# bqqbarbhg/rtk

Hardware: AMD Instinct MI355X
Metric: Mrays/sec (primary, closest-hit) on 1M-tri scene (higher is better)
Workload: dtype f32; 1 GPU; config2: 1M-tri soup (seed 1, spread 0.02), 4096x4096 coherent pinhole primary rays; bvh=gpu-lbvh, bvh_nodes=462584, launch=persistent, ray_order=as given, parallelism=ray-batch shards x1, BVH replicated

## Files before the change

include/rtk_amd.h:

```cpp
#ifndef RTK_AMD_H
#define RTK_AMD_H

#include "rtk.h"

#ifdef __cplusplus
extern "C" {
#endif

enum {
	RTK_AMD_OK = 0,
	RTK_AMD_ERR_NO_DEVICE = -1,
	RTK_AMD_ERR_BAD_ARG = -2,
	RTK_AMD_ERR_OOM = -3,
	RTK_AMD_ERR_HIP = -4,
	RTK_AMD_ERR_BAD_SCENE = -5,
	RTK_AMD_ERR_UNSUPPORTED = -6,
};

const char *rtk_amd_last_error(void);
int rtk_amd_device_count(void);
int rtk_amd_set_device(int device);

typedef struct rtk_dev_scene rtk_dev_scene;

// ... 137 lines not shown
typedef struct rtk_dev_filter {
	uint32_t struct_size;
	uint32_t mesh_mask_bits;
	const uint32_t *d_mesh_mask;
	const uint32_t *d_ignore_prim;
	const rtk_hit_record *d_after;
} rtk_dev_filter;
int rtk_dev_trace_rays_filtered(const rtk_dev_scene *ds, const rtk_ray *d_rays, size_t n,
	rtk_hit_record *d_hits, const rtk_dev_filter *filter, const rtk_trace_opts *opts, void *stream);
int rtk_dev_trace_rays_any_filtered(const rtk_dev_scene *ds, const rtk_ray *d_rays, size_t n,
	uint8_t *d_occluded, const rtk_dev_filter *filter, const rtk_trace_opts *opts, void *stream);
int rtk_dev_trace_status(const rtk_dev_scene *ds, void *stream);

int rtk_dev_detect_image(const rtk_dev_scene *ds, const rtk_ray *d_rays, size_t n, uint32_t *width, uint32_t *height, void *stream);

int rtk_dev_trace_rays_counted(const rtk_dev_scene *ds, const rtk_ray *d_rays, size_t n,
	rtk_hit_record *d_hits, const rtk_trace_opts *opts, rtk_trace_counters *out);

int rtk_dev_trace_rays_any_counted(const rtk_dev_scene *ds, const rtk_ray *d_rays, size_t n,
	uint8_t *d_occluded, const rtk_trace_opts *opts, rtk_trace_counters *out);

typedef struct rtk_packet_counters {
	uint64_t tiles;
	uint64_t pairs;
	uint64_t node_steps;
	uint64_t triangles_fetched;
	uint64_t triangle_group_tests;
	uint64_t tiles_handed_back;
	uint64_t handed_back_node_steps;
	uint64_t handed_back_triangle_steps;
} rtk_packet_counters;
int rtk_dev_trace_rays_packet_counted(const rtk_dev_scene *ds, const rtk_ray *d_rays, size_t n,
	rtk_hit_record *d_hits, const rtk_trace_opts *opts, rtk_packet_counters *out);

typedef struct rtk_mgpu rtk_mgpu;
void rtk_amd_shard_range(size_t n, int rank, int num_shards, size_t *first, size_t *count);
rtk_mgpu *rtk_mgpu_create(const int *devices, int num_devices);
void rtk_mgpu_destroy(rtk_mgpu *m);
int rtk_mgpu_num_devices(const rtk_mgpu *m);
const rtk_dev_scene *rtk_mgpu_scene(const rtk_mgpu *m, int index);
int rtk_mgpu_build(rtk_mgpu *m, const rtk_scene_desc *desc);
int rtk_mgpu_upload(rtk_mgpu *m, const rtk_scene *scene);
int rtk_mgpu_refit(rtk_mgpu *m, const rtk_scene_desc *desc);
int rtk_mgpu_refit_meshes(rtk_mgpu *m, const rtk_scene_desc *desc, const uint32_t *mesh_ids, size_t num_ids);
int rtk_mgpu_build_placed(rtk_mgpu *m, const rtk_scene_desc *desc, const rtk_placement *placements);
int rtk_mgpu_refit_placed(rtk_mgpu *m, const rtk_scene_desc *desc, const rtk_placement *placements);
int rtk_mgpu_refit_meshes_placed(rtk_mgpu *m, const rtk_scene_desc *desc, const rtk_placement *placements,
                                 const uint32_t *mesh_ids, size_t num_ids);
int rtk_mgpu_split_leaves(rtk_mgpu *m, uint32_t max_leaf);
int rtk_mgpu_rebuild(rtk_mgpu *m);
int rtk_mgpu_trace_rays(rtk_mgpu *m, const rtk_ray *rays, size_t n, rtk_hit_record *records, const rtk_trace_opts *opts);
int rtk_mgpu_trace_rays_device(rtk_mgpu *m, const rtk_ray *const *d_rays, const size_t *counts, rtk_hit_record *const *d_records,
	rtk_hit_record *d_gathered, int root_index, const rtk_trace_opts *opts);
int rtk_mgpu_trace_rays_device_striped(rtk_mgpu *m, const rtk_ray *const *d_rays, const size_t *counts, rtk_hit_record *const *d_records,
	rtk_hit_record *const *d_striped, const rtk_trace_opts *opts);
void rtk_mgpu_striped_segment(const size_t *counts, int num_shards, int shard, int stripe, size_t *first, size_t *count);

size_t rtk_trace_rays(const rtk_scene *scene, const rtk_ray *rays, size_t n, rtk_hit *hits, uint8_t *hit_mask);
size_t rtk_trace_rays_filter(const rtk_scene *scene, const rtk_ray *rays, size_t n, rtk_hit *hits, uint8_t *hit_mask,
	rtk_filter_fn *filter, void *filter_user);
void rtk_amd_forget_scene(const rtk_scene *scene);

#ifdef __cplusplus
}
#endif
#endif
// ... 1 lines not shown
```

rtk_amd/api.py:

```python
import ctypes as C
import os

import numpy as np

from .types import (HIT_DTYPE, HIT_RECORD_DTYPE, RAY_DTYPE, MeshSet, Placement, SceneDesc, SceneHeader, placement_array)

HERE = os.path.dirname(os.path.abspath(__file__))
LIB_PATH = os.environ.get("RTK_AMD_LIB") or os.path.join(HERE, "librtk_amd.so")

RTK_TRACE_STATIC = 1
RTK_TRACE_NO_PACKET = 2
RTK_TRACE_SORT_RAYS = 4
RTK_TRACE_EXACT_NODES = 8
RTK_TRACE_NO_ASM = 16


class RtkError(RuntimeError):
    pass


class SceneInfo(C.Structure):
    _fields_ = [("num_triangles", C.c_uint64), ("num_meshes", C.c_uint64), ("num_nodes", C.c_uint64),
                ("node_bytes", C.c_uint64), ("triangle_bytes", C.c_uint64), ("total_device_bytes", C.c_uint64),
                ("max_depth", C.c_uint32), ("stack_entries", C.c_uint32), ("build_ms", C.c_double)]
# ... 40 lines not shown


class TraceOpts(C.Structure):
    _fields_ = [("struct_size", C.c_uint32), ("flags", C.c_uint32), ("image_width", C.c_uint32),
                ("image_height", C.c_uint32), ("refill_min", C.c_uint32), ("blocks_per_cu", C.c_uint32),
                ("node_exit", C.c_uint32)]


class DevFilter(C.Structure):
    _fields_ = [("struct_size", C.c_uint32), ("mesh_mask_bits", C.c_uint32), ("d_mesh_mask", C.c_void_p),
                ("d_ignore_prim", C.c_void_p), ("d_after", C.c_void_p)]


FILTER_FN = C.CFUNCTYPE(C.c_bool, C.c_void_p, C.c_void_p, C.c_void_p)


class TraceCounters(C.Structure):
    _fields_ = [("rays", C.c_uint64), ("nodes", C.c_uint64), ("leaves", C.c_uint64),
                ("triangles", C.c_uint64), ("hits", C.c_uint64), ("stack_spills", C.c_uint64),
                ("wave_node_steps", C.c_uint64), ("wave_triangle_steps", C.c_uint64), ("wave_rays", C.c_uint64)]

    def as_dict(self):
        return {k: int(getattr(self, k)) for k, _ in self._fields_}


class PacketCounters(C.Structure):
    _fields_ = [("tiles", C.c_uint64), ("pairs", C.c_uint64), ("node_steps", C.c_uint64), ("triangles_fetched", C.c_uint64),
                ("triangle_group_tests", C.c_uint64), ("tiles_handed_back", C.c_uint64),
                ("handed_back_node_steps", C.c_uint64), ("handed_back_triangle_steps", C.c_uint64)]

    def as_dict(self):
        return {k: int(getattr(self, k)) for k, _ in self._fields_}


RTK_H_SYMBOLS = ["rtk_start_build", "rtk_run_task", "rtk_get_build_size", "rtk_finish_build_to",
                 "rtk_finish_build", "rtk_build_scene", "rtk_free_scene", "rtk_trace_ray", "rtk_trace_ray_filter"]
RTK_AMD_H_SYMBOLS = ["rtk_amd_last_error", "rtk_amd_device_count", "rtk_amd_set_device",
                     "rtk_dev_scene_upload", "rtk_dev_scene_build", "rtk_dev_scene_free", "rtk_dev_scene_get_info",
                     "rtk_dev_scene_mesh_base", "rtk_dev_scene_primitive_order", "rtk_dev_scene_export_size", "rtk_dev_scene_export",
                     "rtk_dev_trace_rays", "rtk_dev_trace_rays_any", "rtk_dev_expand_hits",
                     "rtk_dev_trace_rays_counted", "rtk_dev_trace_rays_any_counted", "rtk_dev_trace_rays_packet_counted", "rtk_dev_detect_image", "rtk_trace_rays", "rtk_amd_forget_scene",
                     "rtk_dev_scene_validate", "rtk_amd_release_workspace", "rtk_dev_scene_upload_buffer",
                     "rtk_dev_trace_rays_filtered", "rtk_dev_trace_rays_any_filtered", "rtk_dev_trace_status",
                     "rtk_trace_rays_filter", "rtk_amd_shard_range", "rtk_mgpu_create", "rtk_mgpu_destroy", "rtk_mgpu_num_devices",
                     "rtk_mgpu_scene", "rtk_mgpu_build", "rtk_mgpu_upload", "rtk_mgpu_trace_rays", "rtk_mgpu_trace_rays_device",
                     "rtk_amd_set_builder", "rtk_amd_get_builder", "rtk_amd_set_per_ray",
                     "rtk_mgpu_trace_rays_device_striped", "rtk_mgpu_striped_segment",
                     "rtk_dev_scene_refit", "rtk_dev_scene_last_refit_ms", "rtk_mgpu_refit",
                     "rtk_dev_scene_refit_meshes", "rtk_dev_scene_last_refit_nodes", "rtk_mgpu_refit_meshes",
                     "rtk_dev_scene_quality", "rtk_dev_scene_split_leaves", "rtk_mgpu_split_leaves",
                     "rtk_dev_scene_rebuild", "rtk_mgpu_rebuild",
                     "rtk_dev_scene_build_placed", "rtk_dev_scene_refit_placed", "rtk_dev_scene_refit_meshes_placed",
                     "rtk_mgpu_build_placed", "rtk_mgpu_refit_placed", "rtk_mgpu_refit_meshes_placed"]

_lib = None


def lib():
    global _lib
    if _lib is not None:
        return _lib
    if not os.path.exists(LIB_PATH):
        raise RtkError("%s not found: build it with `make -C rtk_amd/csrc` (or __graft_entry__.build()); "
                       "there is no CPU fallback" % LIB_PATH)
    import torch
    L = C.CDLL(LIB_PATH)
    L.rtk_amd_last_error.restype = C.c_char_p
    L.rtk_amd_device_count.restype = C.c_int
    L.rtk_amd_set_device.argtypes = [C.c_int]
    L.rtk_dev_scene_upload.restype = C.c_void_p
    L.rtk_dev_scene_upload.argtypes = [C.c_void_p]
    L.rtk_dev_scene_build.restype = C.c_void_p
    L.rtk_dev_scene_build.argtypes = [C.POINTER(SceneDesc)]
    L.rtk_dev_scene_free.argtypes = [C.c_void_p]
    L.rtk_dev_scene_get_info.argtypes = [C.c_void_p, C.POINTER(SceneInfo)]
    L.rtk_dev_scene_mesh_base.argtypes = [C.c_void_p, C.c_void_p, C.c_size_t]
    L.rtk_dev_scene_primitive_order.restype = C.c_longlong
    L.rtk_dev_scene_primitive_order.argtypes = [C.c_void_p, C.c_void_p, C.c_size_t]
    L.rtk_dev_scene_export_size.restype = C.c_size_t
    L.rtk_dev_scene_export_size.argtypes = [C.c_void_p]
    L.rtk_dev_scene_export.restype = C.c_void_p
    L.rtk_dev_scene_export.argtypes = [C.c_void_p, C.c_void_p, C.c_size_t]
    L.rtk_dev_trace_rays.argtypes = [C.c_void_p, C.c_void_p, C.c_size_t, C.c_void_p, C.POINTER(TraceOpts), C.c_void_p]
    L.rtk_dev_trace_rays_any.argtypes = [C.c_void_p, C.c_void_p, C.c_size_t, C.c_void_p, C.POINTER(TraceOpts), C.c_void_p]
    L.rtk_dev_expand_hits.argtypes = [C.c_void_p, C.c_void_p, C.c_size_t, C.c_void_p, C.c_void_p, C.c_void_p]
    L.rtk_dev_trace_rays_packet_counted.argtypes = [C.c_void_p, C.c_void_p, C.c_size_t, C.c_void_p, C.POINTER(TraceOpts), C.POINTER(PacketCounters)]
    L.rtk_dev_trace_rays_counted.argtypes = [C.c_void_p, C.c_void_p, C.c_size_t, C.c_void_p, C.POINTER(TraceOpts),
                                             C.POINTER(TraceCounters)]
    L.rtk_dev_trace_rays_any_counted.argtypes = [C.c_void_p, C.c_void_p, C.c_size_t, C.c_void_p, C.POINTER(TraceOpts),
                                                 C.POINTER(TraceCounters)]
    L.rtk_trace_rays.restype = C.c_size_t
    L.rtk_trace_rays.argtypes = [C.c_void_p, C.c_void_p, C.c_size_t, C.c_void_p, C.c_void_p]
    L.rtk_amd_forget_scene.argtypes = [C.c_void_p]
    L.rtk_dev_scene_validate.argtypes = [C.c_void_p, C.POINTER(SceneCheck)]
    L.rtk_dev_scene_upload_buffer.restype = C.c_void_p
    L.rtk_dev_scene_upload_buffer.argtypes = [C.c_void_p, C.c_size_t]
    L.rtk_dev_trace_rays_filtered.argtypes = [C.c_void_p, C.c_void_p, C.c_size_t, C.c_void_p, C.POINTER(DevFilter),
                                              C.POINTER(TraceOpts), C.c_void_p]
    L.rtk_dev_trace_rays_any_filtered.argtypes = [C.c_void_p, C.c_void_p, C.c_size_t, C.c_void_p, C.POINTER(DevFilter),
                                                  C.POINTER(TraceOpts), C.c_void_p]
    L.rtk_dev_trace_status.argtypes = [C.c_void_p, C.c_void_p]
    L.rtk_trace_rays_filter.restype = C.c_size_t
    L.rtk_trace_rays_filter.argtypes = [C.c_void_p, C.c_void_p, C.c_size_t, C.c_void_p, C.c_void_p, C.c_void_p, C.c_void_p]
    L.rtk_amd_shard_range.restype = None
    L.rtk_amd_shard_range.argtypes = [C.c_size_t, C.c_int, C.c_int, C.POINTER(C.c_size_t), C.POINTER(C.c_size_t)]
    L.rtk_mgpu_create.restype = C.c_void_p
    L.rtk_mgpu_create.argtypes = [C.POINTER(C.c_int), C.c_int]
    L.rtk_mgpu_destroy.restype = None
    L.rtk_mgpu_destroy.argtypes = [C.c_void_p]
    L.rtk_mgpu_num_devices.argtypes = [C.c_void_p]
    L.rtk_mgpu_scene.restype = C.c_void_p
    L.rtk_mgpu_scene.argtypes = [C.c_void_p, C.c_int]
    L.rtk_mgpu_build.argtypes = [C.c_void_p, C.POINTER(SceneDesc)]
    L.rtk_mgpu_upload.argtypes = [C.c_void_p, C.c_void_p]
    L.rtk_mgpu_refit.restype = C.c_int
    L.rtk_mgpu_refit.argtypes = [C.c_void_p, C.POINTER(SceneDesc)]
    L.rtk_dev_scene_refit.restype = C.c_int
    L.rtk_dev_scene_refit.argtypes = [C.c_void_p, C.POINTER(SceneDesc), C.c_void_p]
    L.rtk_dev_scene_last_refit_ms.restype = C.c_double
# ... 342 lines not shown
            d_rays = to_device(rays)
        d_occ = torch.empty(n, dtype=torch.uint8, device="cuda")
        ctr = TraceCounters()
        torch.cuda.synchronize()
        _check(lib().rtk_dev_trace_rays_any_counted(self.handle, C.c_void_p(d_rays.data_ptr()), n, C.c_void_p(d_occ.data_ptr()),
                                                    C.byref(opts) if opts is not None else None, C.byref(ctr)),
               "rtk_dev_trace_rays_any_counted")
        return d_occ.cpu().numpy().astype(bool), ctr.as_dict()

    def trace_counted(self, rays, opts=None):
        torch = _torch()
        if hasattr(rays, "data_ptr"):
            d_rays, n = rays, rays.numel() * rays.element_size() // 32
        else:
            rays = np.ascontiguousarray(rays)
            n = rays.shape[0]
            d_rays = to_device(rays)
        d_rec = torch.empty(n * 16, dtype=torch.uint8, device="cuda")
        ctr = TraceCounters()
        torch.cuda.synchronize()
        _check(lib().rtk_dev_trace_rays_counted(self.handle, C.c_void_p(d_rays.data_ptr()), n, C.c_void_p(d_rec.data_ptr()),
                                                C.byref(opts) if opts is not None else None, C.byref(ctr)),
               "rtk_dev_trace_rays_counted")
        return d_rec.cpu().numpy().view(HIT_RECORD_DTYPE), ctr.as_dict()


    def detect_image(self, rays):
        rays = np.ascontiguousarray(rays)
        d_rays = to_device(rays)
        w, h = C.c_uint32(0), C.c_uint32(0)
        _check(lib().rtk_dev_detect_image(self.handle, C.c_void_p(d_rays.data_ptr()), C.c_size_t(rays.shape[0]), C.byref(w), C.byref(h), _stream_ptr()), "rtk_dev_detect_image")
        return int(w.value), int(h.value)

    def trace_packet_counted(self, rays, opts):
        torch = _torch()
        if hasattr(rays, "data_ptr"):
            d_rays, n = rays, rays.numel() * rays.element_size() // 32
        else:
            rays = np.ascontiguousarray(rays)
            n = rays.shape[0]
            d_rays = to_device(rays)
        d_rec = torch.empty(n * 16, dtype=torch.uint8, device="cuda")
        ctr = PacketCounters()
        torch.cuda.synchronize()
        _check(lib().rtk_dev_trace_rays_packet_counted(self.handle, C.c_void_p(d_rays.data_ptr()), n, C.c_void_p(d_rec.data_ptr()),
                                                       C.byref(opts) if opts is not None else None, C.byref(ctr)),
               "rtk_dev_trace_rays_packet_counted")
        return d_rec.cpu().numpy().view(HIT_RECORD_DTYPE), ctr.as_dict()



def build_scene(meshes):
    _torch()
    ms = meshes if isinstance(meshes, MeshSet) else MeshSet(meshes)
    p = lib().rtk_build_scene(C.byref(ms.desc))
    if not p:
        raise RtkError("rtk_build_scene failed: " + last_error())
    return p, ms


def free_scene(scene_ptr):
    lib().rtk_free_scene(C.c_void_p(scene_ptr))


def scene_bytes(scene_ptr):
    hdr = SceneHeader.from_address(scene_ptr)
# ... 41 lines not shown
```

rtk_amd/csrc/rtk_capi.hip:

```cpp
#include "rtk_dev.h"
#include "rtk_trace_plan.h"

#include <algorithm>
#include "rtk_layout_check.h"

#include <stdarg.h>
#include <stdio.h>
#include <stdlib.h>
#include <string.h>

#include <chrono>
#include <atomic>
#include <mutex>
#include <unordered_map>


static thread_local char g_error[512] = "";

void rtk_set_error(const char *fmt, ...)
{
	va_list ap;
	va_start(ap, fmt);
	vsnprintf(g_error, sizeof(g_error), fmt, ap);
	va_end(ap);
// ... 107 lines not shown
}

extern "C" int rtk_dev_trace_rays_filtered(const rtk_dev_scene *ds, const rtk_ray *d_rays, size_t n,
	rtk_hit_record *d_hits, const rtk_dev_filter *filter, const rtk_trace_opts *opts, void *stream)
{
	return rtk_launch_trace(ds, d_rays, n, d_hits, nullptr, opts, (hipStream_t)stream, false, nullptr, filter);
}

extern "C" int rtk_dev_trace_rays_any_filtered(const rtk_dev_scene *ds, const rtk_ray *d_rays, size_t n,
	uint8_t *d_occluded, const rtk_dev_filter *filter, const rtk_trace_opts *opts, void *stream)
{
	return rtk_launch_trace(ds, d_rays, n, nullptr, d_occluded, opts, (hipStream_t)stream, true, nullptr, filter);
}

extern "C" int rtk_dev_trace_rays_counted(const rtk_dev_scene *ds, const rtk_ray *d_rays, size_t n,
	rtk_hit_record *d_hits, const rtk_trace_opts *opts, rtk_trace_counters *out)
{
	if (!out) { rtk_set_error("rtk_dev_trace_rays_counted: NULL counters"); return RTK_AMD_ERR_BAD_ARG; }
	return rtk_launch_trace(ds, d_rays, n, d_hits, nullptr, opts, nullptr, false, out);
}

extern "C" int rtk_dev_trace_rays_any_counted(const rtk_dev_scene *ds, const rtk_ray *d_rays, size_t n,
	uint8_t *d_occluded, const rtk_trace_opts *opts, rtk_trace_counters *out)
{
	if (!out) { rtk_set_error("rtk_dev_trace_rays_any_counted: NULL counters"); return RTK_AMD_ERR_BAD_ARG; }
	return rtk_launch_trace(ds, d_rays, n, nullptr, d_occluded, opts, nullptr, true, out);
}

extern "C" int rtk_dev_trace_rays_packet_counted(const rtk_dev_scene *ds, const rtk_ray *d_rays, size_t n,
	rtk_hit_record *d_hits, const rtk_trace_opts *opts, rtk_packet_counters *out)
{
	if (!out) { rtk_set_error("rtk_dev_trace_rays_packet_counted: NULL counters"); return RTK_AMD_ERR_BAD_ARG; }
	return rtk_launch_trace(ds, d_rays, n, d_hits, nullptr, opts, nullptr, false, nullptr, nullptr, nullptr, nullptr, 0, out);
}

extern "C" int rtk_dev_detect_image(const rtk_dev_scene *ds, const rtk_ray *d_rays, size_t n, uint32_t *width, uint32_t *height, void *stream)
{
	if (!ds || !width || !height || (!d_rays && n)) { rtk_set_error("rtk_dev_detect_image: NULL argument"); return RTK_AMD_ERR_BAD_ARG; }
	return rtk_detect_image(ds, d_rays, n, (hipStream_t)stream, width, height);
}

extern "C" int rtk_dev_trace_status(const rtk_dev_scene *ds, void *stream)
{
	return rtk_trace_status(ds, (hipStream_t)stream);
}

extern "C" int rtk_dev_expand_hits(const rtk_dev_scene *ds, const rtk_hit_record *d_records, size_t n,
	rtk_hit *d_hits, uint8_t *d_mask, void *stream)
{
	return rtk_launch_expand(ds, d_records, n, d_hits, d_mask, (hipStream_t)stream);
}


namespace {

const size_t STRIPE = 4096;

uint64_t hash_words(const void *data, size_t n, uint64_t h)
{
	const unsigned char *p = static_cast<const unsigned char *>(data);
	size_t i = 0;
	for (; i + 8 <= n; i += 8) { uint64_t w; memcpy(&w, p + i, 8); h = (h ^ w) * 0x9e3779b97f4a7c15ull; h ^= h >> 29; }
	for (; i < n; i++) { h = (h ^ p[i]) * 0x100000001b3ull; }
	return h;
}

// ... 551 lines not shown
```

rtk_amd/csrc/rtk_dev.h:

```cpp
#pragma once

#include <hip/hip_runtime.h>
#include <stdint.h>
#include <chrono>
#include <mutex>
#include <optional>
#include <vector>

#include "rtk.h"
#include "rtk_amd.h"
#include "rtk_carve.h"
#include "rtk_node.h"
#include "rtk_scene_mem.h"

#define RTK_MAX_DEVICES 64
#define RTK_TRI_LAST 1u
#define RTK_QUEUES 8
#define RTK_QUEUE_WORD(q) (16 + 16 * (q))
#define RTK_COUNTER_WORDS (16 + 16 * RTK_QUEUES)
#define RTK_ERROR_WORD RTK_COUNTER_WORDS

#ifndef RTK_TRI_STRIDE
#define RTK_TRI_STRIDE 48
#endif
// ... 171 lines not shown
int rtk_blob_to_host_bvh(const rtk_scene *scene, size_t avail, HostBvh *out);
rtk_dev_scene *rtk_dev_scene_from_host_bvh(const HostBvh &h);

int rtk_quantize_nodes(rtk_dev_scene *ds, hipStream_t stream, const DevNode *src = nullptr, DevNodeQ *dst = nullptr, float bound_hint = 0.0f,
	uint32_t only_first = 0xffffffffu, bool keep_consts = false, bool readback = true);
int rtk_scene_consts(rtk_dev_scene *ds, hipStream_t stream);
int rtk_quantize_node_list(rtk_dev_scene *ds, hipStream_t stream, const uint32_t *list, const uint32_t *d_count);
void rtk_quantize_finish(rtk_dev_scene *ds);

struct WorkspaceLoan {
	int device = -1;
	char *base = nullptr;
	WorkspaceLoan() = default;
	WorkspaceLoan(const WorkspaceLoan &) = delete;
	WorkspaceLoan &operator=(const WorkspaceLoan &) = delete;
	~WorkspaceLoan() { release(); }
	bool take(int device, size_t bytes);
	void release();
};
bool rtk_is_device_ptr(const void *p);
void rtk_export_forget(const rtk_dev_scene *ds);
void rtk_sah_costs(float *cost_node, float *cost_tri);

size_t rtk_sort_scratch_words(uint32_t n);
bool rtk_sort_pairs_async(unsigned long long *keys_a, unsigned long long *keys_b, uint32_t *vals_a, uint32_t *vals_b,
	uint32_t n, uint32_t key_bits, uint32_t *scratch, hipStream_t stream);
bool rtk_sort_words_async(unsigned long long *keys_a, unsigned long long *keys_b, uint32_t n, uint32_t first_bit, uint32_t last_bit,
	uint32_t *scratch, hipStream_t stream);

int rtk_launch_trace(const rtk_dev_scene *ds, const rtk_ray *d_rays, size_t n, rtk_hit_record *d_hits,
	uint8_t *d_occluded, const rtk_trace_opts *opts, hipStream_t stream, bool any_hit, rtk_trace_counters *counted,
	const rtk_dev_filter *filter = nullptr, rtk_hit_record *d_cand = nullptr, uint32_t *d_cand_count = nullptr, uint32_t cand_k = 0,
	rtk_packet_counters *pk_counted = nullptr);
int rtk_detect_image(const rtk_dev_scene *ds, const rtk_ray *d_rays, size_t n, hipStream_t stream, uint32_t *w_out, uint32_t *h_out);
int rtk_trace_status(const rtk_dev_scene *ds, hipStream_t stream);
void rtk_scratch_free(LaunchScratch *s);
void rtk_scene_drop_stream(rtk_dev_scene *ds, hipStream_t stream);
int rtk_launch_trace_one(const rtk_dev_scene *ds, const rtk_ray *d_ray, rtk_hit *d_hit, uint8_t *d_mask, hipStream_t stream,
	unsigned long long *h_status, uint32_t ticket);
int rtk_launch_expand(const rtk_dev_scene *ds, const rtk_hit_record *d_records, size_t n, rtk_hit *d_hits,
	uint8_t *d_mask, hipStream_t stream, unsigned long long *h_status = nullptr, uint32_t ticket = 0);
```

rtk_amd/csrc/rtk_trace.hip:

```cpp
#include "rtk_dev.h"

#include <algorithm>
#include "rtk_trace_shared.h"

#include <math.h>
#include <stdio.h>
#include <stdlib.h>

#include <mutex>

#include "rtk_trace_lane.h"

#define RTK_PUSH(e_)                                                                                        \
	do {                                                                                                    \
		if (sp < LDS_STACK) { stk[sp][lane] = (e_); sp++; }                                                 \
		else if (sp - LDS_STACK < p.spill_cap) {                                                            \
			p.spill[(size_t)(sp - LDS_STACK) * p.spill_stride + glane] = (e_); sp++; if (COUNT) c_spills++; \
		} else p.counter[RTK_ERROR_WORD] = 1ull;                                                            \
	} while (0)

#define RTK_REF_RETRY 0xfffffffeu
#define RTK_POP()                                                                                           \
	do {                                                                                                    \
		if (sp == 0u) top = RTK_REF_NONE;                                                                   \
// ... 1123 lines not shown
	p.dynamic = plan.dynamic;
	p.refill_min = plan.refill_min;
	p.node_exit = plan.node_exit;
	p.image_w = plan.image_w;
	p.image_h = plan.image_h;
	p.tile_blocks = plan.tile_blocks;

	std::lock_guard<std::mutex> lock(ds->scratch_mutex);
	LaunchScratch *sc = scratch_for(ds, stream);
	if (!sc) return RTK_AMD_ERR_OOM;
	int rc = grow_scratch(sc, plan, n, stream);
	if (rc != RTK_AMD_OK) return rc;
	p.spill = sc->d_spill;
	p.spill_stride = (uint32_t)(plan.spill_cap ? sc->spill_lanes : 0);
	p.spill_cap = (uint32_t)plan.spill_cap;
	p.counter = sc->d_counter;
	if (plan.sort_rays && (rc = enqueue_sort(ds, sc, d_rays, n, knobs, stream, &p.perm)) != RTK_AMD_OK) return rc;
	if ((plan.dynamic || plan.packet || counted) && !plan.entries) RTK_HIP_CHECK(hipMemsetAsync(sc->d_counter, 0, RTK_COUNTER_WORDS * sizeof(unsigned long long), stream), RTK_AMD_ERR_HIP);
	if (plan.entries) {
		rtk_packet_entries_launch(p, (PkBlockEntries *)sc->d_entries, ds->tree.bound_abs > 1.0f ? ds->tree.bound_abs : 1.0f, knobs.entry_target, knobs.entry_levels, stream);
		p.entries = (const PkBlockEntries *)sc->d_entries;
	}
	if (plan.hot) rc = enqueue_packet_hot(ds, sc, p, plan, any_hit, pk_counted != nullptr, stream);
	else if (plan.packet) rtk_packet_launch(p, (unsigned)plan.grid, stream, counted != nullptr);
	else if (plan.lane_hot) rc = enqueue_lane_hot(ds, sc, p, plan, any_hit, o.refill_given, knobs, stream);
	else hipLaunchKernelGGL(trace_variant(plan.variant), dim3((unsigned)plan.grid), dim3(BLOCK_THREADS), 0, stream, p);
	if (rc != RTK_AMD_OK) return rc;
	RTK_HIP_CHECK(hipGetLastError(), RTK_AMD_ERR_HIP);
	if (pk_counted && (rc = read_packet_counters(sc, n, stream, pk_counted)) != RTK_AMD_OK) return rc;
	if (counted) return read_counters(sc, stream, counted);
	return RTK_AMD_OK;
}

int rtk_trace_status(const rtk_dev_scene *ds_c, hipStream_t stream)
{
	rtk_dev_scene *ds = const_cast<rtk_dev_scene *>(ds_c);
	if (!ds) { rtk_set_error("rtk_dev_trace_status: NULL scene"); return RTK_AMD_ERR_BAD_ARG; }
	unsigned long long *word = nullptr;
	{
		std::lock_guard<std::mutex> lock(ds->scratch_mutex);
		for (LaunchScratch *s : ds->scratch) if (s->stream == stream) { word = s->d_counter + RTK_ERROR_WORD; break; }
	}
	if (!word) {
		RTK_HIP_CHECK(hipStreamSynchronize(stream), RTK_AMD_ERR_HIP);
		return RTK_AMD_OK;
	}
	unsigned long long e = 0;
	RTK_HIP_CHECK(hipMemcpyAsync(&e, word, sizeof(e), hipMemcpyDeviceToHost, stream), RTK_AMD_ERR_HIP);
	RTK_HIP_CHECK(hipStreamSynchronize(stream), RTK_AMD_ERR_HIP);
	if (e) {
		(void)hipMemsetAsync(word, 0, sizeof(e), stream);
		rtk_set_error("rtk_dev_trace: traversal stack overflow (corrupted scene)");
		return RTK_AMD_ERR_BAD_SCENE;
	}
	return RTK_AMD_OK;
}

void rtk_scene_drop_stream(rtk_dev_scene *ds, hipStream_t stream)
{
	if (!ds) return;
	std::lock_guard<std::mutex> lock(ds->scratch_mutex);
	for (size_t i = 0; i < ds->scratch.size();) {
		if (ds->scratch[i]->stream == stream) { rtk_scratch_free(ds->scratch[i]); ds->scratch.erase(ds->scratch.begin() + (long)i); } else i++;
	}
}

// ... 37 lines not shown
```

rtk_amd/csrc/rtk_trace_packet.hip:

```cpp
#include "rtk_dev.h"
#include "rtk_trace_shared.h"

#include <math.h>

#define PK_LDS_STACK 16
#define PK_WAVE_STACK 64
#ifndef PK_MIN_WAVES
#define PK_MIN_WAVES 7
#endif

typedef int i32x16 __attribute__((ext_vector_type(16)));
typedef int i32x8 __attribute__((ext_vector_type(8)));
typedef int i32x4 __attribute__((ext_vector_type(4)));
typedef float f32x4 __attribute__((ext_vector_type(4)));

__device__ __forceinline__ float asf(int v) { return __int_as_float(v); }

struct PkNode { i32x4 nx, fx, ny, fy, nz, fz, ch; int ord; };
__device__ __forceinline__ void s_load_node(const char *addr, uint32_t onx, uint32_t ofx, uint32_t ony, uint32_t ofy,
	uint32_t onz, uint32_t ofz, uint32_t oord, PkNode &n)
{
	asm volatile(
		"s_load_dwordx4 %0, %8, %9\n\t"
		"s_load_dwordx4 %1, %8, %10\n\t"
		"s_load_dwordx4 %2, %8, %11\n\t"
		"s_load_dwordx4 %3, %8, %12\n\t"
		"s_load_dwordx4 %4, %8, %13\n\t"
		"s_load_dwordx4 %5, %8, %14\n\t"
		"s_load_dwordx4 %6, %8, 0x60\n\t"
		"s_load_dword %7, %8, %15\n\t"
		"s_waitcnt lgkmcnt(0)"
		: "=&s"(n.nx), "=&s"(n.fx), "=&s"(n.ny), "=&s"(n.fy), "=&s"(n.nz), "=&s"(n.fz), "=&s"(n.ch), "=&s"(n.ord)
		: "s"(addr), "s"(onx), "s"(ofx), "s"(ony), "s"(ofy), "s"(onz), "s"(ofz), "s"(oord)
		: "memory");
// ... 446 lines not shown
						top = (uint32_t)__builtin_amdgcn_readfirstlane((int)ent->e[ent_next].ref);
						ent_next++;
						took = live_m != 0ull;
					}
					if (!took) break;
					continue;
				}
				top = (uint32_t)__builtin_amdgcn_readlane((int)stack, (int)sp);
			}
		}

		if (overflow && lane == 0) p.counter[RTK_ERROR_WORD] = 1ull;
		if (alive) {
			if (p.occluded) p.occluded[ray_index] = L.prim != RTK_PRIM_NONE ? 1 : 0;
			else {
				f32x4 rec;
				rec.x = L.t; rec.y = L.u; rec.z = L.v; rec.w = __uint_as_float(L.prim);
				__builtin_nontemporal_store(rec, reinterpret_cast<f32x4 *>(p.hits + ray_index));
			}
			if (COUNT) {
				atomicAdd(p.counter + 1, 1ull);
				atomicAdd(p.counter + 2, (unsigned long long)c_nodes);
				atomicAdd(p.counter + 3, (unsigned long long)c_leaves);
				atomicAdd(p.counter + 4, (unsigned long long)c_tris);
				atomicAdd(p.counter + 5, L.prim != RTK_PRIM_NONE ? 1ull : 0ull);
				atomicAdd(p.counter + 6, (unsigned long long)c_spills);
			}
		}
	}
}


namespace {
struct PkBeam { float olo[3], ohi[3], rlo[3], rhi[3], m[3], tmin; uint32_t neg; };

__device__ __forceinline__ bool pk_beam_child(const DevNode &nd, int k, const PkBeam &b, float &tlo)
{
	const float lo[3] = { nd.bx[0][k], nd.by[0][k], nd.bz[0][k] }, hi[3] = { nd.bx[1][k], nd.by[1][k], nd.bz[1][k] };
	float n = b.tmin, f = INFINITY;
#pragma unroll
	for (int a = 0; a < 3; a++) {
		const bool neg = (b.neg >> a) & 1u;
		const float pn = neg ? hi[a] : lo[a], pf = neg ? lo[a] : hi[a];
		const float n0 = (pn - b.olo[a]) * b.rlo[a], n1 = (pn - b.olo[a]) * b.rhi[a], n2 = (pn - b.ohi[a]) * b.rlo[a], n3 = (pn - b.ohi[a]) * b.rhi[a];
		const float f0 = (pf - b.olo[a]) * b.rlo[a], f1 = (pf - b.olo[a]) * b.rhi[a], f2 = (pf - b.ohi[a]) * b.rlo[a], f3 = (pf - b.ohi[a]) * b.rhi[a];
		n = fmaxf(n, fminf(fminf(n0, n1), fminf(n2, n3)) - b.m[a]);
		f = fminf(f, fmaxf(fmaxf(f0, f1), fmaxf(f2, f3)) + b.m[a]);
	}
	tlo = n;
	return n <= f;
}

__device__ __forceinline__ float wave_min(float v) { for (int o = 32; o > 0; o >>= 1) v = fminf(v, __shfl_xor(v, o)); return v; }
__device__ __forceinline__ float wave_max(float v) { for (int o = 32; o > 0; o >>= 1) v = fmaxf(v, __shfl_xor(v, o)); return v; }

#define PK_FRONTIER 128
__global__ void __launch_bounds__(64) rtk_packet_entries_kernel(const DevNode *nodes, const rtk_ray *rays, uint32_t image_w, uint32_t blocks_per_row,
	float bound_abs, uint32_t target, uint32_t max_levels, PkBlockEntries *out, unsigned long long *counter)
{
	__shared__ uint32_t s_ref[2][PK_FRONTIER];
	if (blockIdx.x == 0) for (uint32_t w = threadIdx.x; w < (uint32_t)RTK_COUNTER_WORDS; w += 64u) counter[w] = 0ull;
	__shared__ float s_t[2][PK_FRONTIER];
	__shared__ uint32_t s_out_ref[PK_MAX_ENTRIES];
	__shared__ float s_out_t[PK_MAX_ENTRIES];
	const uint32_t lane = threadIdx.x, blk = blockIdx.x;
	const uint32_t bx = blk % blocks_per_row, by = blk / blocks_per_row;
	PkBeam b;
	bool ok = true;
	uint32_t s_and = 7u, s_or = 0u;
	float tmin = INFINITY;
	for (int a = 0; a < 3; a++) { b.olo[a] = INFINITY; b.ohi[a] = -INFINITY; b.rlo[a] = INFINITY; b.rhi[a] = -INFINITY; }
	if (lane < 9u) {
		const uint32_t x = (lane % 3u) == 0u ? 0u : ((lane % 3u) == 1u ? 31u : 63u);
		const uint32_t y = (lane / 3u) == 0u ? 0u : ((lane / 3u) == 1u ? 31u : 63u);
		const rtk_ray r = rays[(size_t)(by * 64u + y) * image_w + bx * 64u + x];
		const float o[3] = { r.origin.x, r.origin.y, r.origin.z }, d[3] = { r.direction.x, r.direction.y, r.direction.z };
		uint32_t sg = 0;
		for (int a = 0; a < 3; a++) {
			const float rd = 1.0f / d[a];
			ok = ok && fabsf(o[a]) < 0x1p19f && fabsf(rd) > 0x1p-100f && fabsf(rd) < 0x1p100f;
			b.olo[a] = o[a]; b.ohi[a] = o[a];
			b.rlo[a] = rd; b.rhi[a] = rd;
			sg |= (__float_as_uint(d[a]) >> 31) << a;
		}
		ok = ok && r.min_t == r.min_t && r.max_t == r.max_t;
		tmin = r.min_t;
		s_and = sg; s_or = sg;
	}
	for (int o = 32; o > 0; o >>= 1) { s_and &= __shfl_xor(s_and, o); s_or |= __shfl_xor(s_or, o); }
	ok = __builtin_amdgcn_ballot_w64(!ok) == 0ull && s_and == s_or && bound_abs < 0x1p19f;
	for (int a = 0; a < 3; a++) {
		b.olo[a] = wave_min(b.olo[a]); b.ohi[a] = wave_max(b.ohi[a]); b.rlo[a] = wave_min(b.rlo[a]); b.rhi[a] = wave_max(b.rhi[a]);
		b.rlo[a] -= 0x1p-22f * fabsf(b.rlo[a]); b.rhi[a] += 0x1p-22f * fabsf(b.rhi[a]);
		b.m[a] = 0x1p-21f * (fmaxf(fabsf(b.rlo[a]), fabsf(b.rhi[a])) * (fmaxf(fabsf(b.olo[a]), fabsf(b.ohi[a])) + bound_abs));
	}
	b.tmin = wave_min(tmin);
	b.neg = s_or;
	PkBlockEntries *e = out + blk;
	if (lane == 0) {
		for (int a = 0; a < 3; a++) { e->olo[a] = b.olo[a]; e->ohi[a] = b.ohi[a]; e->rlo[a] = b.rlo[a]; e->rhi[a] = b.rhi[a]; }
		e->pad[0] = __float_as_uint(b.tmin); e->pad[1] = 0u; e->pad[2] = 0u;
		if (!ok) e->count = 0u;
	}
	if (!ok) return;
	uint32_t n_cur = 1u, n_out = 0u, cur = 0u;
	bool over = false;
	if (lane == 0) { s_ref[0][0] = 0u; s_t[0][0] = b.tmin; }
	__syncthreads();
	for (int level = 0; level < (int)max_levels && n_cur != 0u; level++) {
		if (level > 0 && n_out + n_cur >= target) break;
		uint32_t n_next = 0u;
		for (uint32_t base = 0; base < n_cur; base += 64u) {
			const bool have = base + lane < n_cur;
			const uint32_t ref = have ? s_ref[cur][base + lane] : 0u;
			const float t_self = have ? s_t[cur][base + lane] : 0.0f;
			const DevNode nd = nodes[ref];
			bool pass[4], leaf_below = false;
			float tlo[4];
#pragma unroll
			for (int k = 0; k < 4; k++) {
				tlo[k] = 0.0f;
				pass[k] = have && nd.child[k] != RTK_REF_NONE && pk_beam_child(nd, k, b, tlo[k]);
				leaf_below = leaf_below || (pass[k] && (nd.child[k] & RTK_REF_LEAF) != 0u);
			}
			const bool list_self = have && leaf_below;
			const unsigned long long below = (1ull << lane) - 1ull;
			const unsigned long long m_out = __builtin_amdgcn_ballot_w64(list_self);
			if (list_self) {
				const uint32_t at = n_out + (uint32_t)__popcll(m_out & below);
				if (at < PK_MAX_ENTRIES) { s_out_ref[at] = ref; s_out_t[at] = t_self; }
			}
			n_out += (uint32_t)__popcll(m_out);
#pragma unroll
			for (int k = 0; k < 4; k++) {
				const bool push = pass[k] && !list_self;
				const unsigned long long m_next = __builtin_amdgcn_ballot_w64(push);
				if (push) {
					const uint32_t at = n_next + (uint32_t)__popcll(m_next & below);
					if (at < PK_FRONTIER) { s_ref[cur ^ 1u][at] = nd.child[k]; s_t[cur ^ 1u][at] = tlo[k]; }
				}
				n_next += (uint32_t)__popcll(m_next);
			}
		}
		over = over || n_out > PK_MAX_ENTRIES || n_next > PK_FRONTIER;
		if (over) break;
		__syncthreads();
		cur ^= 1u;
		n_cur = n_next;
	}
	if (!over) {
		for (uint32_t i = lane; i < n_cur; i += 64u) if (n_out + i < PK_MAX_ENTRIES) { s_out_ref[n_out + i] = s_ref[cur][i]; s_out_t[n_out + i] = s_t[cur][i]; }
		n_out += n_cur;
		over = n_out > PK_MAX_ENTRIES;
	}
	__syncthreads();
	if (over) { if (lane == 0) e->count = 0u; return; }
	if (lane < n_out) {
		const float t = s_out_t[lane];
		uint32_t rank = 0;
		for (uint32_t j = 0; j < n_out; j++) { const float tj = s_out_t[j]; rank += (tj < t || (tj == t && j < lane)) ? 1u : 0u; }
		e->e[rank].ref = s_out_ref[lane];
		e->e[rank].tlo = t;
	}
	if (lane == 0) e->count = n_out;
}
}

void rtk_packet_entries_launch(const TraceParams &p, PkBlockEntries *out, float bound_abs, unsigned target, unsigned max_levels, hipStream_t stream)
{
	const uint32_t bpr = p.image_w >> 6, rows = p.image_h >> 6;
	hipLaunchKernelGGL(rtk_packet_entries_kernel, dim3(bpr * rows), dim3(64), 0, stream, p.sc.nodes, p.rays, p.image_w, bpr, bound_abs, target, max_levels, out, p.counter);
}

#include "rtk_packet_hot_image.h"

AsmModule &rtk_packet_module()
{
	static const AsmKernel table[NUM_PACKET_KERNELS] = {
		{ "rtk_packet_hot", 7 },
		{ "rtk_packet_beam", 8 },
		{ "rtk_packet_beam2", 7 },
		{ "rtk_packet_count2", 0 },
		{ "rtk_packet_any2", 0 },
	};
	static AsmModule m(rtk_packet_hot_image, table, NUM_PACKET_KERNELS, "rtk_dev_trace: the assembly packet kernel is not loaded");
	return m;
}

int rtk_packet_occupancy(bool counted)
{
	int nb = 0;
	hipError_t e = counted ? hipOccupancyMaxActiveBlocksPerMultiprocessor(&nb, rtk_trace_packet_kernel<true>, TRACE_BLOCK_THREADS, 0)
	                       : hipOccupancyMaxActiveBlocksPerMultiprocessor(&nb, rtk_trace_packet_kernel<false>, TRACE_BLOCK_THREADS, 0);
	return (e == hipSuccess && nb >= 1) ? nb : 1;
// ... 8 lines not shown
```

Baseline: 25240 Mrays/s.

## Parallelize packet-entries beam traversal per child lane with DPP reductions

Restructures the packet-entries kernel so each lane tests one child of a node (four lanes per node, 16 nodes per pass) rather than one lane testing all four children of a node. Wave-wide shuffle reductions become DPP row reductions followed by readfirstlane, the child test uses a cheaper sign-selected interval formula, and the final rank sort reads values through readlane instead of shared memory. It also adds a debug entry point and a Python dtype for inspecting the per-block entries. Risks: the row-0 reduction only covers lanes within one DPP row, so the beam bounds may ignore other lanes, and the cheaper child test may be less conservative than the four-corner version.

```diff
diff --git a/include/rtk_amd.h b/include/rtk_amd.h
--- a/include/rtk_amd.h
+++ b/include/rtk_amd.h
@@ -193,6 +193,9 @@
 } rtk_packet_counters;
 int rtk_dev_trace_rays_packet_counted(const rtk_dev_scene *ds, const rtk_ray *d_rays, size_t n,
 	rtk_hit_record *d_hits, const rtk_trace_opts *opts, rtk_packet_counters *out);
+
+int rtk_dev_debug_packet_entries(const rtk_dev_scene *ds, const rtk_ray *d_rays, uint32_t image_w, uint32_t image_h,
+	uint32_t target, uint32_t max_levels, void *host_out);
 
 typedef struct rtk_mgpu rtk_mgpu;
 void rtk_amd_shard_range(size_t n, int rank, int num_shards, size_t *first, size_t *count);
diff --git a/rtk_amd/api.py b/rtk_amd/api.py
--- a/rtk_amd/api.py
+++ b/rtk_amd/api.py
@@ -96,6 +96,10 @@
     def as_dict(self):
         return {k: int(getattr(self, k)) for k, _ in self._fields_}
 
+
+PACKET_ENTRIES_DTYPE = np.dtype([("olo", "<f4", (3,)), ("ohi", "<f4", (3,)), ("rlo", "<f4", (3,)), ("rhi", "<f4", (3,)), ("count", "<u4"), ("tmin", "<f4"),
+                                 ("pad", "<u4", (2,)), ("e", [("ref", "<u4"), ("tlo", "<f4")], (56,))])
+assert PACKET_ENTRIES_DTYPE.itemsize == 512
 
 RTK_H_SYMBOLS = ["rtk_start_build", "rtk_run_task", "rtk_get_build_size", "rtk_finish_build_to",
                  "rtk_finish_build", "rtk_build_scene", "rtk_free_scene", "rtk_trace_ray", "rtk_trace_ray_filter"]
@@ -103,7 +107,7 @@
                      "rtk_dev_scene_upload", "rtk_dev_scene_build", "rtk_dev_scene_free", "rtk_dev_scene_get_info",
                      "rtk_dev_scene_mesh_base", "rtk_dev_scene_primitive_order", "rtk_dev_scene_export_size", "rtk_dev_scene_export",
                      "rtk_dev_trace_rays", "rtk_dev_trace_rays_any", "rtk_dev_expand_hits",
-                     "rtk_dev_trace_rays_counted", "rtk_dev_trace_rays_any_counted", "rtk_dev_trace_rays_packet_counted", "rtk_dev_detect_image", "rtk_trace_rays", "rtk_amd_forget_scene",
+                     "rtk_dev_trace_rays_counted", "rtk_dev_trace_rays_any_counted", "rtk_dev_trace_rays_packet_counted", "rtk_dev_debug_packet_entries", "rtk_dev_detect_image", "rtk_trace_rays", "rtk_amd_forget_scene",
                      "rtk_dev_scene_validate", "rtk_amd_release_workspace", "rtk_dev_scene_upload_buffer",
                      "rtk_dev_trace_rays_filtered", "rtk_dev_trace_rays_any_filtered", "rtk_dev_trace_status",
                      "rtk_trace_rays_filter", "rtk_amd_shard_range", "rtk_mgpu_create", "rtk_mgpu_destroy", "rtk_mgpu_num_devices",
@@ -149,6 +153,8 @@
     L.rtk_dev_trace_rays_any.argtypes = [C.c_void_p, C.c_void_p, C.c_size_t, C.c_void_p, C.POINTER(TraceOpts), C.c_void_p]
     L.rtk_dev_expand_hits.argtypes = [C.c_void_p, C.c_void_p, C.c_size_t, C.c_void_p, C.c_void_p, C.c_void_p]
     L.rtk_dev_trace_rays_packet_counted.argtypes = [C.c_void_p, C.c_void_p, C.c_size_t, C.c_void_p, C.POINTER(TraceOpts), C.POINTER(PacketCounters)]
+    L.rtk_dev_debug_packet_entries.restype = C.c_int
+    L.rtk_dev_debug_packet_entries.argtypes = [C.c_void_p, C.c_void_p, C.c_uint32, C.c_uint32, C.c_uint32, C.c_uint32, C.c_void_p]
     L.rtk_dev_trace_rays_counted.argtypes = [C.c_void_p, C.c_void_p, C.c_size_t, C.c_void_p, C.POINTER(TraceOpts),
                                              C.POINTER(TraceCounters)]
     L.rtk_dev_trace_rays_any_counted.argtypes = [C.c_void_p, C.c_void_p, C.c_size_t, C.c_void_p, C.POINTER(TraceOpts),
@@ -557,6 +563,16 @@
         _check(lib().rtk_dev_detect_image(self.handle, C.c_void_p(d_rays.data_ptr()), C.c_size_t(rays.shape[0]), C.byref(w), C.byref(h), _stream_ptr()), "rtk_dev_detect_image")
         return int(w.value), int(h.value)
 
+    def debug_packet_entries(self, rays, width, height, target=26, max_levels=8):
+        torch = _torch()
+        d_rays = rays if hasattr(rays, "data_ptr") else to_device(np.ascontiguousarray(rays))
+        assert d_rays.numel() * d_rays.element_size() == width * height * 32
+        out = np.zeros((width // 64) * (height // 64), dtype=PACKET_ENTRIES_DTYPE)
+        torch.cuda.synchronize()
+        _check(lib().rtk_dev_debug_packet_entries(self.handle, C.c_void_p(d_rays.data_ptr()), width, height, target, max_levels,
+                                                  C.c_void_p(out.ctypes.data)), "rtk_dev_debug_packet_entries")
+        return out
+
     def trace_packet_counted(self, rays, opts):
         torch = _torch()
         if hasattr(rays, "data_ptr"):
diff --git a/rtk_amd/csrc/rtk_capi.hip b/rtk_amd/csrc/rtk_capi.hip
--- a/rtk_amd/csrc/rtk_capi.hip
+++ b/rtk_amd/csrc/rtk_capi.hip
@@ -163,6 +163,12 @@
 {
 	if (!out) { rtk_set_error("rtk_dev_trace_rays_packet_counted: NULL counters"); return RTK_AMD_ERR_BAD_ARG; }
 	return rtk_launch_trace(ds, d_rays, n, d_hits, nullptr, opts, nullptr, false, nullptr, nullptr, nullptr, nullptr, 0, out);
+}
+
+extern "C" int rtk_dev_debug_packet_entries(const rtk_dev_scene *ds, const rtk_ray *d_rays, uint32_t image_w, uint32_t image_h,
+	uint32_t target, uint32_t max_levels, void *host_out)
+{
+	return rtk_debug_packet_entries(ds, d_rays, image_w, image_h, target, max_levels, host_out);
 }
 
 extern "C" int rtk_dev_detect_image(const rtk_dev_scene *ds, const rtk_ray *d_rays, size_t n, uint32_t *width, uint32_t *height, void *stream)
diff --git a/rtk_amd/csrc/rtk_dev.h b/rtk_amd/csrc/rtk_dev.h
--- a/rtk_amd/csrc/rtk_dev.h
+++ b/rtk_amd/csrc/rtk_dev.h
@@ -227,6 +227,7 @@
 	uint8_t *d_occluded, const rtk_trace_opts *opts, hipStream_t stream, bool any_hit, rtk_trace_counters *counted,
 	const rtk_dev_filter *filter = nullptr, rtk_hit_record *d_cand = nullptr, uint32_t *d_cand_count = nullptr, uint32_t cand_k = 0,
 	rtk_packet_counters *pk_counted = nullptr);
+int rtk_debug_packet_entries(const rtk_dev_scene *ds, const rtk_ray *d_rays, uint32_t image_w, uint32_t image_h, uint32_t target, uint32_t max_levels, void *host_out);
 int rtk_detect_image(const rtk_dev_scene *ds, const rtk_ray *d_rays, size_t n, hipStream_t stream, uint32_t *w_out, uint32_t *h_out);
 int rtk_trace_status(const rtk_dev_scene *ds, hipStream_t stream);
 void rtk_scratch_free(LaunchScratch *s);
diff --git a/rtk_amd/csrc/rtk_entries_rule.h b/rtk_amd/csrc/rtk_entries_rule.h
--- /dev/null
+++ b/rtk_amd/csrc/rtk_entries_rule.h
@@ -0,0 +1,45 @@
+#pragma once
+
+#include <math.h>
+#include <stdint.h>
+
+#if defined(__HIPCC__)
+#define RTK_ENTRIES_FN __host__ __device__ inline
+#else
+#define RTK_ENTRIES_FN static inline
+#endif
+
+struct RtkEntriesBeam { float olo[3], ohi[3], rlo[3], rhi[3], m[3], tmin; uint32_t neg; };
+
+RTK_ENTRIES_FN bool rtk_entries_child_full(const float lo[3], const float hi[3], const RtkEntriesBeam &b, float *tlo)
+{
+	float n = b.tmin, f = INFINITY;
+	for (int a = 0; a < 3; a++) {
+		const bool neg = (b.neg >> a) & 1u;
+		const float pn = neg ? hi[a] : lo[a], pf = neg ? lo[a] : hi[a];
+		const float n0 = (pn - b.olo[a]) * b.rlo[a], n1 = (pn - b.olo[a]) * b.rhi[a], n2 = (pn - b.ohi[a]) * b.rlo[a], n3 = (pn - b.ohi[a]) * b.rhi[a];
+		const float f0 = (pf - b.olo[a]) * b.rlo[a], f1 = (pf - b.olo[a]) * b.rhi[a], f2 = (pf - b.ohi[a]) * b.rlo[a], f3 = (pf - b.ohi[a]) * b.rhi[a];
+		n = fmaxf(n, fminf(fminf(n0, n1), fminf(n2, n3)) - b.m[a]);
+		f = fminf(f, fmaxf(fmaxf(f0, f1), fmaxf(f2, f3)) + b.m[a]);
+	}
+	*tlo = n;
+	return n <= f;
+}
+
+RTK_ENTRIES_FN bool rtk_entries_child(const float lo[3], const float hi[3], const RtkEntriesBeam &b, float *tlo)
+{
+	float n = b.tmin, f = INFINITY;
+#if defined(__HIPCC__)
+#pragma unroll
+#endif
+	for (int a = 0; a < 3; a++) {
+		const bool neg = (b.neg >> a) & 1u;
+		const float pn = neg ? hi[a] : lo[a], pf = neg ? lo[a] : hi[a];
+		const float dn = pn - (neg ? b.olo[a] : b.ohi[a]), df = pf - (neg ? b.ohi[a] : b.olo[a]);
+		const float nr = dn * (dn >= 0.0f ? b.rlo[a] : b.rhi[a]), fr = df * (df >= 0.0f ? b.rhi[a] : b.rlo[a]);
+		n = fmaxf(n, nr - b.m[a]);
+		f = fminf(f, fr + b.m[a]);
+	}
+	*tlo = n;
+	return n <= f;
+}
diff --git a/rtk_amd/csrc/rtk_trace.hip b/rtk_amd/csrc/rtk_trace.hip
--- a/rtk_amd/csrc/rtk_trace.hip
+++ b/rtk_amd/csrc/rtk_trace.hip
@@ -1179,6 +1179,36 @@
 	return RTK_AMD_OK;
 }
 
+int rtk_debug_packet_entries(const rtk_dev_scene *ds_c, const rtk_ray *d_rays, uint32_t image_w, uint32_t image_h, uint32_t target, uint32_t max_levels, void *host_out)
+{
+	rtk_dev_scene *ds = const_cast<rtk_dev_scene *>(ds_c);
+	if (!ds || !d_rays || !host_out) { rtk_set_error("rtk_dev_debug_packet_entries: NULL argument"); return RTK_AMD_ERR_BAD_ARG; }
+	if (image_w == 0 || image_h == 0 || (image_w & 63u) || (image_h & 63u) || (unsigned long long)image_w * image_h > 0xffffffffull) {
+		rtk_set_error("rtk_dev_debug_packet_entries: %u x %u is not an image of whole 64x64-pixel blocks", image_w, image_h);
+		return RTK_AMD_ERR_BAD_ARG;
+	}
+	if (!on_scene_device(ds, "rtk_dev_debug_packet_entries")) return RTK_AMD_ERR_BAD_ARG;
+	if (ds->view.num_nodes == 0) { rtk_set_error("rtk_dev_debug_packet_entries: the scene has no nodes"); return RTK_AMD_ERR_BAD_ARG; }
+	const hipStream_t stream = nullptr;
+	std::lock_guard<std::mutex> lock(ds->scratch_mutex);
+	LaunchScratch *sc = scratch_for(ds, stream);
+	if (!sc) return RTK_AMD_ERR_OOM;
+	const size_t nblk = (size_t)(image_w >> 6) * (image_h >> 6);
+	const int rc = grow(&sc->d_entries, &sc->entries_capacity, nblk, nblk * sizeof(PkBlockEntries), stream);
+	if (rc != RTK_AMD_OK) return rc;
+	TraceParams p = {};
+	p.sc = ds->view;
+	p.rays = d_rays;
+	p.image_w = image_w;
+	p.image_h = image_h;
+	p.counter = sc->d_counter;
+	rtk_packet_entries_launch(p, (PkBlockEntries *)sc->d_entries, ds->tree.bound_abs > 1.0f ? ds->tree.bound_abs : 1.0f, target, max_levels, stream);
+	RTK_HIP_CHECK(hipGetLastError(), RTK_AMD_ERR_HIP);
+	RTK_HIP_CHECK(hipMemcpyAsync(host_out, sc->d_entries, nblk * sizeof(PkBlockEntries), hipMemcpyDeviceToHost, stream), RTK_AMD_ERR_HIP);
+	RTK_HIP_CHECK(hipStreamSynchronize(stream), RTK_AMD_ERR_HIP);
+	return RTK_AMD_OK;
+}
+
 int rtk_trace_status(const rtk_dev_scene *ds_c, hipStream_t stream)
 {
 	rtk_dev_scene *ds = const_cast<rtk_dev_scene *>(ds_c);
diff --git a/rtk_amd/csrc/rtk_trace_packet.hip b/rtk_amd/csrc/rtk_trace_packet.hip
--- a/rtk_amd/csrc/rtk_trace_packet.hip
+++ b/rtk_amd/csrc/rtk_trace_packet.hip
@@ -1,5 +1,6 @@
 #include "rtk_dev.h"
 #include "rtk_trace_shared.h"
+#include "rtk_entries_rule.h"
 
 #include <math.h>
 
@@ -512,27 +513,13 @@
 
 
 namespace {
-struct PkBeam { float olo[3], ohi[3], rlo[3], rhi[3], m[3], tmin; uint32_t neg; };
-
-__device__ __forceinline__ bool pk_beam_child(const DevNode &nd, int k, const PkBeam &b, float &tlo)
-{
-	const float lo[3] = { nd.bx[0][k], nd.by[0][k], nd.bz[0][k] }, hi[3] = { nd.bx[1][k], nd.by[1][k], nd.bz[1][k] };
-	float n = b.tmin, f = INFINITY;
-#pragma unroll
-	for (int a = 0; a < 3; a++) {
-		const bool neg = (b.neg >> a) & 1u;
-		const float pn = neg ? hi[a] : lo[a], pf = neg ? lo[a] : hi[a];
-		const float n0 = (pn - b.olo[a]) * b.rlo[a], n1 = (pn - b.olo[a]) * b.rhi[a], n2 = (pn - b.ohi[a]) * b.rlo[a], n3 = (pn - b.ohi[a]) * b.rhi[a];
-		const float f0 = (pf - b.olo[a]) * b.rlo[a], f1 = (pf - b.olo[a]) * b.rhi[a], f2 = (pf - b.ohi[a]) * b.rlo[a], f3 = (pf - b.ohi[a]) * b.rhi[a];
-		n = fmaxf(n, fminf(fminf(n0, n1), fminf(n2, n3)) - b.m[a]);
-		f = fminf(f, fmaxf(fmaxf(f0, f1), fmaxf(f2, f3)) + b.m[a]);
-	}
-	tlo = n;
-	return n <= f;
-}
-
-__device__ __forceinline__ float wave_min(float v) { for (int o = 32; o > 0; o >>= 1) v = fminf(v, __shfl_xor(v, o)); return v; }
-__device__ __forceinline__ float wave_max(float v) { for (int o = 32; o > 0; o >>= 1) v = fmaxf(v, __shfl_xor(v, o)); return v; }
+template <int CTRL> __device__ __forceinline__ uint32_t pk_dpp(uint32_t v) { return (uint32_t)__builtin_amdgcn_update_dpp(0, (int)v, CTRL, 0xf, 0xf, false); }
+template <int CTRL> __device__ __forceinline__ float pk_dpp(float v) { return __uint_as_float(pk_dpp<CTRL>(__float_as_uint(v))); }
+#define PK_ROW_REDUCE(v, OP) do { v = OP(v, pk_dpp<0xB1>(v)); v = OP(v, pk_dpp<0x4E>(v)); v = OP(v, pk_dpp<0x141>(v)); v = OP(v, pk_dpp<0x140>(v)); } while (0)
+__device__ __forceinline__ uint32_t pk_and(uint32_t a, uint32_t b) { return a & b; }
+__device__ __forceinline__ uint32_t pk_or(uint32_t a, uint32_t b) { return a | b; }
+__device__ __forceinline__ float row0_min(float v) { PK_ROW_REDUCE(v, fminf); return __uint_as_float((uint32_t)__builtin_amdgcn_readfirstlane((int)__float_as_uint(v))); }
+__device__ __forceinline__ float row0_max(float v) { PK_ROW_REDUCE(v, fmaxf); return __uint_as_float((uint32_t)__builtin_amdgcn_readfirstlane((int)__float_as_uint(v))); }
 
 #define PK_FRONTIER 128
 __global__ void __launch_bounds__(64) rtk_packet_entries_kernel(const DevNode *nodes, const rtk_ray *rays, uint32_t image_w, uint32_t blocks_per_row,
@@ -545,7 +532,10 @@
 	__shared__ float s_out_t[PK_MAX_ENTRIES];
 	const uint32_t lane = threadIdx.x, blk = blockIdx.x;
 	const uint32_t bx = blk % blocks_per_row, by = blk / blocks_per_row;
-	PkBeam b;
+	const uint32_t k = lane & 3u, q = lane >> 2;
+	float lo[3] = { nodes[0].bx[0][k], nodes[0].by[0][k], nodes[0].bz[0][k] }, hi[3] = { nodes[0].bx[1][k], nodes[0].by[1][k], nodes[0].bz[1][k] };
+	uint32_t child = nodes[0].child[k];
+	RtkEntriesBeam b;
 	bool ok = true;
 	uint32_t s_and = 7u, s_or = 0u;
 	float tmin = INFINITY;
@@ -567,14 +557,16 @@
 		tmin = r.min_t;
 		s_and = sg; s_or = sg;
 	}
-	for (int o = 32; o > 0; o >>= 1) { s_and &= __shfl_xor(s_and, o); s_or |= __shfl_xor(s_or, o); }
+	PK_ROW_REDUCE(s_and, pk_and);
+	PK_ROW_REDUCE(s_or, pk_or);
+	s_and = (uint32_t)__builtin_amdgcn_readfirstlane((int)s_and); s_or = (uint32_t)__builtin_amdgcn_readfirstlane((int)s_or);
 	ok = __builtin_amdgcn_ballot_w64(!ok) == 0ull && s_and == s_or && bound_abs < 0x1p19f;
 	for (int a = 0; a < 3; a++) {
-		b.olo[a] = wave_min(b.olo[a]); b.ohi[a] = wave_max(b.ohi[a]); b.rlo[a] = wave_min(b.rlo[a]); b.rhi[a] = wave_max(b.rhi[a]);
+		b.olo[a] = row0_min(b.olo[a]); b.ohi[a] = row0_max(b.ohi[a]); b.rlo[a] = row0_min(b.rlo[a]); b.rhi[a] = row0_max(b.rhi[a]);
 		b.rlo[a] -= 0x1p-22f * fabsf(b.rlo[a]); b.rhi[a] += 0x1p-22f * fabsf(b.rhi[a]);
 		b.m[a] = 0x1p-21f * (fmaxf(fabsf(b.rlo[a]), fabsf(b.rhi[a])) * (fmaxf(fabsf(b.olo[a]), fabsf(b.ohi[a])) + bound_abs));
 	}
-	b.tmin = wave_min(tmin);
+	b.tmin = row0_min(tmin);
 	b.neg = s_or;
 	PkBlockEntries *e = out + blk;
 	if (lane == 0) {
@@ -586,41 +578,39 @@
 	uint32_t n_cur = 1u, n_out = 0u, cur = 0u;
 	bool over = false;
 	if (lane == 0) { s_ref[0][0] = 0u; s_t[0][0] = b.tmin; }
-	__syncthreads();
+	const unsigned long long below = (1ull << lane) - 1ull;
 	for (int level = 0; level < (int)max_levels && n_cur != 0u; level++) {
 		if (level > 0 && n_out + n_cur >= target) break;
 		uint32_t n_next = 0u;
-		for (uint32_t base = 0; base < n_cur; base += 64u) {
-			const bool have = base + lane < n_cur;
-			const uint32_t ref = have ? s_ref[cur][base + lane] : 0u;
-			const float t_self = have ? s_t[cur][base + lane] : 0.0f;
-			const DevNode nd = nodes[ref];
-			bool pass[4], leaf_below = false;
-			float tlo[4];
-#pragma unroll
-			for (int k = 0; k < 4; k++) {
-				tlo[k] = 0.0f;
-				pass[k] = have && nd.child[k] != RTK_REF_NONE && pk_beam_child(nd, k, b, tlo[k]);
-				leaf_below = leaf_below || (pass[k] && (nd.child[k] & RTK_REF_LEAF) != 0u);
-			}
-			const bool list_self = have && leaf_below;
-			const unsigned long long below = (1ull << lane) - 1ull;
-			const unsigned long long m_out = __builtin_amdgcn_ballot_w64(list_self);
-			if (list_self) {
+		for (uint32_t base = 0; base < n_cur; base += 16u) {
+			const bool have = base + q < n_cur;
+			uint32_t ref = 0u;
+			float t_self = b.tmin;
+			if (level > 0) {
+				if (have) { ref = s_ref[cur][base + q]; t_self = s_t[cur][base + q]; }
+				const DevNode &nd = nodes[ref];
+				lo[0] = nd.bx[0][k]; lo[1] = nd.by[0][k]; lo[2] = nd.bz[0][k];
+				hi[0] = nd.bx[1][k]; hi[1] = nd.by[1][k]; hi[2] = nd.bz[1][k];
+				child = nd.child[k];
+			}
+			float tlo = 0.0f;
+			const bool pass = have && child != RTK_REF_NONE && rtk_entries_child(lo, hi, b, &tlo);
+			const unsigned long long m_leaf = __builtin_amdgcn_ballot_w64(pass && (child & RTK_REF_LEAF) != 0u);
+			const bool list_self = ((uint32_t)(m_leaf >> (lane & ~3u)) & 0xfu) != 0u;
+			const bool first = list_self && k == 0u;
+			const unsigned long long m_out = __builtin_amdgcn_ballot_w64(first);
+			if (first) {
 				const uint32_t at = n_out + (uint32_t)__popcll(m_out & below);
 				if (at < PK_MAX_ENTRIES) { s_out_ref[at] = ref; s_out_t[at] = t_self; }
 			}
 			n_out += (uint32_t)__popcll(m_out);
-#pragma unroll
-			for (int k = 0; k < 4; k++) {
-				const bool push = pass[k] && !list_self;
-				const unsigned long long m_next = __builtin_amdgcn_ballot_w64(push);
-				if (push) {
-					const uint32_t at = n_next + (uint32_t)__popcll(m_next & below);
-					if (at < PK_FRONTIER) { s_ref[cur ^ 1u][at] = nd.child[k]; s_t[cur ^ 1u][at] = tlo[k]; }
-				}
-				n_next += (uint32_t)__popcll(m_next);
-			}
+			const bool push = pass && !list_self;
+			const unsigned long long m_next = __builtin_amdgcn_ballot_w64(push);
+			if (push) {
+				const uint32_t at = n_next + (uint32_t)__popcll(m_next & below);
+				if (at < PK_FRONTIER) { s_ref[cur ^ 1u][at] = child; s_t[cur ^ 1u][at] = tlo; }
+			}
+			n_next += (uint32_t)__popcll(m_next);
 		}
 		over = over || n_out > PK_MAX_ENTRIES || n_next > PK_FRONTIER;
 		if (over) break;
@@ -635,11 +625,16 @@
 	}
 	__syncthreads();
 	if (over) { if (lane == 0) e->count = 0u; return; }
-	if (lane < n_out) {
-		const float t = s_out_t[lane];
-		uint32_t rank = 0;
-		for (uint32_t j = 0; j < n_out; j++) { const float tj = s_out_t[j]; rank += (tj < t || (tj == t && j < lane)) ? 1u : 0u; }
-		e->e[rank].ref = s_out_ref[lane];
+	const bool mine = lane < n_out;
+	const float t = mine ? s_out_t[lane] : INFINITY;
+	const uint32_t r_mine = mine ? s_out_ref[lane] : 0u;
+	uint32_t rank = 0;
+	for (uint32_t j = 0; j < n_out; j++) {
+		const float tj = __uint_as_float((uint32_t)__builtin_amdgcn_readlane((int)__float_as_uint(t), (int)j));
+		rank += (tj < t || (tj == t && j < lane)) ? 1u : 0u;
+	}
+	if (mine) {
+		e->e[rank].ref = r_mine;
 		e->e[rank].tlo = t;
 	}
 	if (lane == 0) e->count = n_out;
```

After: 25550 Mrays/s, median of 6. +1.3%, better.
